# LLNL/MuyGPyS

Hardware: AMD Instinct MI355X
Metric: neighborhoods/sec (posterior mean+var) (higher is better)
Workload: dtype f32

## Files before the change

muygpys_amd/csrc/mgp_fused_wave_kernel.h:

```cpp
#pragma once

#include "mgp_wave_common.h"

#define MGP_PHASE(g, bit) ((g).mask & (bit))

#ifndef MGP_F64_SAME_PRIO
#define MGP_F64_SAME_PRIO 0
#endif
#ifndef MGP_DIST_PRIO
#define MGP_DIST_PRIO 1
#endif
#ifndef MGP_PRIO_EARLY_RAISE
#define MGP_PRIO_EARLY_RAISE 0
#endif
#ifndef MGP_W4
#define MGP_W4 0
#endif
#ifndef MGP_PRIO_LATE_DROP
#define MGP_PRIO_LATE_DROP 0
#endif
#ifndef MGP_XCHG_PRIO
#define MGP_XCHG_PRIO 0
#endif
#ifndef MGP_CHOL_PRIO
#define MGP_CHOL_PRIO 2
#endif
#ifndef MGP_LOOKAHEAD
#define MGP_LOOKAHEAD 1
#endif
#ifndef MGP_CHOL_ONE_BLOCK
#define MGP_CHOL_ONE_BLOCK 1
#endif
#ifndef MGP_F64_COV_BATCH
#define MGP_F64_COV_BATCH 5
#endif
#ifndef MGP_OWN_REG
#define MGP_OWN_REG 0
#endif
#ifndef MGP_C4_W3
#define MGP_C4_W3 1
#endif
#ifndef MGP_MODM
#define MGP_MODM 1
#endif
#ifndef MGP_GRAM
#define MGP_GRAM 1
#endif
#ifndef MGP_GRAM64
#define MGP_GRAM64 0
#endif
#ifndef MGP_DMA_ASM
#define MGP_DMA_ASM 1
#endif
#ifndef MGP_DIST_ASM
#define MGP_DIST_ASM 1
#endif
#ifndef MGP_F64_GC
#define MGP_F64_GC 6
#endif
#ifndef MGP_FOLD
#define MGP_FOLD 1
#endif
#ifndef MGP_DLT
#define MGP_DLT 1
#endif
#ifndef MGP_F64_DIST_HALF
#define MGP_F64_DIST_HALF 0
#endif

#ifndef MGP_BWD_COV_BATCH
#define MGP_BWD_COV_BATCH 3
#endif
#ifndef MGP_BWD_SWEEP_LATE
#define MGP_BWD_SWEEP_LATE -1
#endif
#ifndef MGP_BWD_EXP
#define MGP_BWD_EXP 0
#endif
#ifndef MGP_FEAT_EXP
#define MGP_FEAT_EXP 0
#endif

namespace mgp {

struct WaveGeom {
  int q;
  int dst;
  int xs;
  int vec_ok;
  int64_t ntasks;
  int mask;
  int gen_tab;
  float gen_h, gen_lc;
  double gen_h64, gen_lc64, gen_xmin64;
};

struct WaveDims {
  int E, CH, NH, NPL, NG, KS, KMAT, BA, BP, NS, M;
  bool STAT, TRI, MODM;
  bool DLT;
  int NR2, NPAIR, NSL;
};
constexpr int dlt_col_start(int c, int NR2) {
  const int m = c >> 1, b = c & 1;
  return 2 * m * NR2 - m * (m - 1) + b * (NR2 - m);
}
constexpr bool wave_bwd_tailfree(int es, int NP, bool gram, int dst) { return es == 4 && NP == 32 && gram && dst > 32 && dst <= 40; }
constexpr WaveDims wave_dims(int es, int NP, int KFIX, int RFIX, int DFIX, bool COEFF, bool GRAM) {
  WaveDims w{};
  w.E = 16 / es;
  w.CH = 2 * w.E;
  w.NH = 64 / NP;
  w.STAT = KFIX > 0 && RFIX > 0 && DFIX > 0 && !COEFF;
  w.NPL = w.STAT ? KFIX + 1 + RFIX : NP;
  w.NG = (w.NPL + w.E - 1) / w.E;
  w.KS = NP + w.E;
  w.TRI = NP == 64 && !COEFF;
  w.DLT = MGP_DLT && es == 8 && NP == 64 && w.STAT && RFIX >= 1;
  w.NR2 = (w.NPL + 1) / 2;
  w.NPAIR = dlt_col_start(w.NPL, w.NR2);
  w.NSL = (w.NPAIR + 63) / 64;
  w.KMAT = w.TRI ? w.E * ((w.NPL - 1) / w.E + 1) * (w.E * ((w.NPL - 1) / w.E) / 2 + (w.NPL - 1) % w.E) + w.NG * w.E + w.E
                 : NP * w.KS;
  if (w.DLT) w.KMAT = 2 * 64 * w.NSL + 2;
  w.M = NP;
  w.BA = 4;
  w.BP = NP / 8;
  w.MODM = false;
  if (MGP_MODM && w.STAT) {
    const int need = (KFIX + 1) / 2;
    int ba = 4, bp = (need + 3) / 4;
    for (int c = 3; c <= 5; c += 2) {
      const int q = (need + c - 1) / c;
      if (c * q < ba * bp) ba = c, bp = q;
    }
    if (ba * bp + (GRAM ? 2 : 1) <= NP / 2) {
      w.MODM = true;
      w.M = KFIX + 1;
      w.BA = ba;
      w.BP = bp;
    }
  }
  w.NS = w.BA * w.BP;
  return w;
}
constexpr int wave_pair_delta(int s, int BP, int M) {
  const int j = s / BP, p = s % BP + 1, o = j == 0 ? 0 : (j + 1) * BP + 1;
  return ((o - p) % M + M) % M;
}
constexpr bool wave_pair_first(int s, int BP, int M) {
  const int d = wave_pair_delta(s, BP, M);
  if (d == 0) return false;
  for (int t = 0; t < s; ++t) {
    const int e = wave_pair_delta(t, BP, M);
    if (e == d || e == M - d) return false;
  }
  return true;
}
constexpr unsigned long long wave_pair_first_mask(int NS, int BP, int M) {
  unsigned long long m = 0;
  for (int s = 0; s < NS; ++s)
    if (wave_pair_first(s, BP, M)) m |= 1ull << s;
  return m;
}
constexpr unsigned long long wave_pair_half_mask(int NS, int BP, int M) {
  unsigned long long m = 0;
  for (int s = 0; s < NS; ++s)
    if (2 * wave_pair_delta(s, BP, M) == M) m |= 1ull << s;
  return m;
}
constexpr int wave_tile_rows(const WaveDims& w, int NP, int KFIX, int xs) {
  if (!(w.STAT && w.NH == 1)) return w.NH * NP;
  const int spr = xs / w.E, pieces = ((KFIX + 1) * spr + 63) / 64;
  const int covered = (pieces * 64 + spr - 1) / spr;
  const int rows = w.MODM ? w.NPL : NP;
  return covered > rows ? covered : rows;
}
constexpr int wave_gather_pieces(const WaveDims& w, int KFIX, int xs) {
  const int spr = xs / w.E;
  return (w.STAT && w.NH == 1) ? ((KFIX + 1) * spr + 63) / 64 : spr;
}
constexpr int wave_stage_elems(const WaveDims& w) { return w.DLT ? 2 * (32 + 128) : 0; }
#ifndef MGP_RT_W3
#define MGP_RT_W3 1
#endif
constexpr int wave_min_waves(int es, int NP, int KFIX, int RFIX = 0, int DFIX = 0) {
  return es == 4 ? (NP <= 32 ? (KFIX == 30 && MGP_W4 ? 4 : 3) : (MGP_RT_W3 && KFIX == 0 ? 3 : 2))
                 : (NP <= 32 ? 2 : (MGP_C4_W3 && wave_dims(es, NP, KFIX, RFIX, DFIX, false, false).DLT ? 3 : 2));
}

#ifndef MGP_FOLD64
#define MGP_FOLD64 1
#endif
#ifndef MGP_FOLD16
#define MGP_FOLD16 0
#endif
#ifndef MGP_FOLD_F64
#define MGP_FOLD_F64 0
#endif
constexpr bool wave_fold(int es, int NP, int KFIX, int RFIX, int DFIX, bool PIPED, bool COEFF, bool GRAM) {
  return MGP_FOLD && PIPED && KFIX > 0 && RFIX >= 1 && DFIX > 0 && !COEFF && KFIX >= NP / 2 &&
         ((es == 4 && GRAM && (NP == 32 || (NP == 64 && MGP_FOLD64) || (NP == 16 && MGP_FOLD16))) || (es == 8 && NP == 32 && MGP_FOLD_F64));
}
constexpr int wave_colbuf_bytes(int es, int NP, bool fold) {
  const int need = fold ? (64 / (NP / 2)) * NP * es : 64 * es;
  return need > 512 ? need : 512;
}

template <int NPL_>
struct DltMeta {
  static constexpr int NR2 = (NPL_ + 1) / 2;
  static constexpr int NPAIR = dlt_col_start(NPL_, NR2);
  static constexpr int NSL = (NPAIR + 63) / 64;
  int rc[NSL * 64][2];
  constexpr DltMeta() : rc{} {
    int c = 0;
    for (int e = 0; e < NSL * 64; ++e) {
      while (c + 1 < NPL_ && dlt_col_start(c + 1, NR2) <= e) ++c;
      rc[e][0] = e < NPAIR ? 2 * (e - dlt_col_start(c, NR2) + (c >> 1)) : 0;
      rc[e][1] = c;
// ... 114 lines not shown
  const bool nopad = k == q;

  const int64_t ntasks = g.ntasks;
  const int64_t per_xcd = (ntasks + 7) / 8;
  const int xcd = blockIdx.x & 7;
  const int64_t t_hi = (xcd + 1) * per_xcd;
  const int64_t t_end = t_hi < ntasks ? t_hi : ntasks;
  const int64_t t_step = gridDim.x >> 3;

  auto load_index = [&](int task, int h, int i) -> int64_t {
    const int64_t nb0 = (int64_t)task * NH;
    const int hh = (NH > 1 && nb0 + h >= a.b) ? 0 : h;
    const int64_t* row = a.nn_idx + nb0 * k;
    const int64_t* p = row + (hh * k + (i < k ? i : 0));
    if (a.batch_idx != nullptr && i == q) p = a.batch_idx + nb0 + hh;
    return *p;
  };
  auto fix_index = [&](int64_t raw, int task, int h, int i) -> int64_t {
    const int64_t nb0 = (int64_t)task * NH;
    const int hh = (NH > 1 && nb0 + h >= a.b) ? 0 : h;
    if (i < k) return raw;
    if (i == q) return a.batch_idx != nullptr ? raw : nb0 + hh;
    return 0;
  };

  const int64_t task0 = xcd * per_xcd + (blockIdx.x >> 3);

  int g_pos = 0;
  auto seq_gen = [&]() -> int {
    const int64_t ts = task0 + (int64_t)g_pos * t_step;
    ++g_pos;
    return ts < t_end ? (int)ts : -1;
  };
  int task = seq_gen(), t1 = seq_gen(), t2 = -1;
  int64_t next_idx = 0;
  if (task >= 0) next_idx = load_index(task, NH == 1 ? 0 : (int)threadIdx.x / NP, threadIdx.x & (NP - 1));

  constexpr bool PIPE = PIPED;
  static_assert(!PIPED || DFIX <= DCAP, "the pipelined gather stages all features at once");
  const int SPR = xs / E;
  const int C16V = d / E;
  constexpr int GB = 11;
  const unsigned spr_magic = (1u << 20) / (unsigned)SPR + 1u;
  T pre_y = T(0), pre_eps = T(0);
  int64_t pre_idx = 0, pre_tg = 0;
  auto pipe_issue = [&](int task_n, int64_t idx_n, int lane_) {
    const int h = NH == 1 ? 0 : lane_ / NP;
    const int i = lane_ & (NP - 1);
    if constexpr (PACKED)
      rowaddr[lane_] = reinterpret_cast<const T*>(
          (i == q ? static_cast<const char*>(a.packed_q) + idx_n * a.q_stride
                  : static_cast<const char*>(a.packed_nn) + idx_n * a.nn_stride));
    else
      rowaddr[lane_] = (i == q ? feat_q : feat_nn) + idx_n * (int64_t)d;
    pre_idx = idx_n;
    __syncthreads();
    if (MGP_PHASE(g, 1)) {
      const int NPC = wave_gather_pieces(WD, KFIX, xs);
      for (int n0 = 0; n0 < NPC; n0 += GB) {
        const T* src[GB];
#pragma unroll
        for (int u = 0; u < GB; ++u) {
          if (n0 + u < NPC) {
            const unsigned sigma = 64u * (unsigned)(n0 + u) + (unsigned)lane_;
            const unsigned row = (sigma * spr_magic) >> 20;
            const unsigned c = min(sigma - row * (unsigned)SPR, (unsigned)(PACKED ? C16V : C16V - 1));
            src[u] = rowaddr[row] + c * E;
          }
        }
#pragma unroll
        for (int u = 0; u < GB; ++u)
          if (n0 + u < NPC) {
#if MGP_DMA_ASM
            glds16_asm(src[u], smem, (n0 + u) * 1024);
#else
            glds16_lds(src[u], smem, (n0 + u) * 1024);
#endif
          }
      }
    }
    {
      const int64_t nb0 = (int64_t)task_n * NH;
      const int hh = (NH > 1 && nb0 + h >= a.b) ? 0 : h;
      pre_tg = a.targets_batch ? (nb0 + hh) * k + (i < k ? i : 0) : (i < k ? idx_n : 0);
    }
    if (!PACKED || a.targets_batch) pre_y = targets[pre_tg * (int64_t)R];
    if constexpr (BWD) {
      if (a.R > 1) {
        const T* gmp = static_cast<const T*>(a.bwd_gmean);
        const int64_t nbq = (int64_t)task_n * NH + ((NH > 1 && (int64_t)task_n * NH + h >= a.b) ? 0 : h);
        T ys = T(0);
        for (int r = 0; r < a.R; ++r) ys = fma_t(gmp ? gmp[nbq * a.R + r] : T(0), targets[pre_tg * (int64_t)a.R + r], ys);
        pre_y = ys;
      }
    }
    pre_eps = (T)a.noise_scalar;
    if (a.noise_mode != MGP_NOISE_SCALAR) {
      const int64_t nb0 = (int64_t)task_n * NH;
      const int hh = (NH > 1 && nb0 + h >= a.b) ? 0 : h;
      const T* pn = a.noise_mode == MGP_NOISE_TABLE ? noise_dev + (i < k ? idx_n : 0) : noise_dev + nb0 * k + (hh * k + (i < k ? i : 0));
      pre_eps = *pn;
    }
  };
  if (PIPE && task >= 0) {
    pipe_issue(task, fix_index(next_idx, task, NH == 1 ? 0 : (int)threadIdx.x / NP, threadIdx.x & (NP - 1)),
               threadIdx.x);
    if (t1 >= 0) next_idx = load_index(t1, NH == 1 ? 0 : (int)threadIdx.x / NP, threadIdx.x & (NP - 1));
  }

  constexpr bool XPRE = (NP <= 32 || KFIX > 0) && !COEFF;
#ifndef MGP_FOLD_XPK
#define MGP_FOLD_XPK 0
#endif
#ifndef MGP_FOLD_DPRE
#define MGP_FOLD_DPRE 0
#endif
  constexpr bool XPK = XPRE && (NS > 16 || (FOLD && (MGP_FOLD_XPK || sizeof(T) == 8)));
  static_assert(!XPK || NH * KMAT + (BWD ? 4096 : 0) < 65536, "packed exchange offsets are 16-bit");
  int xoff[XPRE ? (XPK ? (NS + 1) / 2 : NS) : 1];
  unsigned xkeep = 0;
  if constexpr (XPRE) {
    const int i0 = threadIdx.x & (NP - 1);
    const int hbase = (NH == 1 ? 0 : (int)threadIdx.x / NP) * KMAT + kmat_base;
    const int dump0 = DLT ? KMAT - 2 : (TRI ? KMAT - E : (NP - 1) * KS + NP);
#pragma unroll
    for (int s = 1; s <= NS; ++s) {
      const int r1 = wrap(i0 + own_offset((s - 1) / BP));
      const int c = wrap(i0 + (s - 1) % BP + 1);
      const int hi = max(r1, c), lo = min(r1, c);
      const int xo = hbase + (hi <= q && hi != lo && i0 < M ? eoff(hi, lo) : dump0);
      if constexpr (XPK) {
        if ((s - 1) % 2 == 0) xoff[(s - 1) / 2] = xo;
        else xoff[(s - 1) / 2] |= xo << 16;
      } else {
        xoff[s - 1] = xo;
      }
      if (lo < k && (hi < k || hi == q)) xkeep |= 1u << (s - 1);
    }
  }

  constexpr bool DPRE = XPRE && DFIX > 0 && NP <= 32 && (!FOLD || MGP_FOLD_DPRE);
  int down[DPRE ? BA : 1], dpar[DPRE ? BP : 1];
  if constexpr (DPRE) {
    const int i0 = threadIdx.x & (NP - 1);
    const int hb = (NH == 1 ? 0 : (int)threadIdx.x / NP) * NP * xs;
#pragma unroll
    for (int j = 0; j < BA; ++j) down[j] = hb + wrap(i0 + own_offset(j)) * xs;
#pragma unroll
    for (int s2 = 1; s2 <= BP; ++s2) dpar[s2 - 1] = hb + wrap(i0 + s2) * xs;
  }
  static_assert(!MODM || XPRE, "the modulo-M pair scheme relies on the per-lane exchange offsets");
  static_assert(!DLT || XPRE, "the dealt layout is written through the per-lane exchange offsets");

  V FL[FOLD ? NG : 1], FS[FOLD ? NGS : 1];
  int fold_sub = 0;
  int fold_task_a = 0;
  for (; task >= 0; task = t1, t1 = t2) {
    int lane = threadIdx.x;
    asm volatile("" : "+v"(lane));
    const int h = NH == 1 ? 0 : lane / NP;
    const int i = lane & (NP - 1);
    T* Xh = tile + h * NP * xs;
    T* Kh = tile + kmat_base + h * KMAT;
    T* colh = TF ? Xh + KFIX * xs : colbuf + h * NP;
    int64_t* idxh = idxbuf + h * NP;
    const int64_t nb0 = (int64_t)task * NH;
    const bool live = nb0 + h < a.b;
    const int hh = live ? h : 0;


    int64_t myidx = 0, mytg = 0;
    T myeps = T(0), myy0 = T(0);
    V myyv = V(0);
    if (PIPE) {
      myidx = pre_idx;
      mytg = pre_tg;
      myy0 = i < k ? pre_y : T(0);
      myeps = pre_eps;
    } else {
      myidx = fix_index(next_idx, task, h, i);
      if (t1 >= 0) next_idx = load_index(t1, h, i);
      __syncthreads();
      idxh[i] = myidx * (int64_t)d;
      mytg = a.targets_batch ? (nb0 + hh) * k + (i < k ? i : 0) : myidx;
      if (i < k) {
        myy0 = targets[mytg * (int64_t)R];
        if (a.noise_mode == MGP_NOISE_SCALAR) myeps = (T)a.noise_scalar;
        else if (a.noise_mode == MGP_NOISE_TABLE) myeps = noise_dev[myidx];
        else myeps = (noise_dev + nb0 * k)[hh * k + i];
      }
    }

    ACC acc[NS];
#pragma unroll
    for (int s = 0; s < NS; ++s) acc[s] = ACC(0);
#if MGP_CHOL_PRIO && MGP_PRIO_LATE_DROP
    __builtin_amdgcn_s_setprio(0);
#endif
#if MGP_DIST_PRIO
    __builtin_amdgcn_s_setprio(sizeof(T) == 4 || MGP_F64_SAME_PRIO ? MGP_DIST_PRIO : MGP_XCHG_PRIO);
#endif

    for (int d0 = 0; d0 < d; d0 += dst) {
      const int w = min(dst, d - d0);
      const int wp = (w + CH - 1) / CH * CH;
      constexpr int ILN = PIPED ? (DSTFIX + 63) / 64 : 1;
      T il_pre[ILN];
      if constexpr (PIPED) {
#pragma unroll
        for (int u = 0; u < ILN; ++u) {
          const int c = u * 64 + lane;
          il_pre[u] = (aniso && c < w) ? T(1) / ls[d0 + c] : T(0);
        }
      }
#if MGP_DMA_ASM
      if (PIPE) lds_dma_wait();
#endif
      __syncthreads();
      MGP_WAVE_T(0)
      if (PIPE) {
        if constexpr (PACKED) {
          if (!a.targets_batch) {
            myyv = *reinterpret_cast<const V*>(Xh + (NPL == NP ? i : min(i, NPL - 1)) * xs + d);
            myy0 = i < k ? myyv[0] : T(0);
          }
        }
        if (wp > w && (NPL == NP || i < NPL)) *reinterpret_cast<V*>(Xh + i * xs + w) = V(0);
      } else if (!MGP_PHASE(g, 1)) {
      } else if (DFIX > 0 || g.vec_ok) {
        const int c16 = w / E, c16p = wp / E;
        const int rpr = NP / c16p;
        const int sub = DFIX > 0 ? i / c16p : (int)(((unsigned)i * ((1u << 16) / (unsigned)c16p + 1u)) >> 16);
        const int c = i - sub * c16p;
        const bool lane_on = sub < rpr;
        constexpr int RPRFIX = NP / (DSTFIX / E);
        constexpr int U = (KFIX > 0 && DFIX > 0) ? (KFIX + RPRFIX - 1) / RPRFIX : 6;
        const int64_t* idxl = idxh + sub;
        T* xdst = Xh + sub * xs + c * E;
        for (int r0 = 0; r0 < k; r0 += U * rpr) {
          V v[U];
#pragma unroll
          for (int u = 0; u < U; ++u) {
            const int row = r0 + u * rpr + sub;
            v[u] = V(0);
            if (lane_on && row < k && c < c16)
              v[u] = *reinterpret_cast<const V*>(feat_nn + idxl[r0 + u * rpr] + d0 + c * E);
          }
#pragma unroll
          for (int u = 0; u < U; ++u) {
            const int row = r0 + u * rpr + sub;
            if (lane_on && row < k) *reinterpret_cast<V*>(xdst + (r0 + u * rpr) * xs) = v[u];
          }
        }
        if (i < c16p) {
          V vq = V(0);
          if (i < c16) vq = *reinterpret_cast<const V*>(feat_q + idxh[q] + d0 + i * E);
          *reinterpret_cast<V*>(Xh + q * xs + i * E) = vq;
        }
        if (!nopad)
          for (int t = i; t < (q - k) * c16p; t += NP) {
            const int row = k + t / c16p;
            *reinterpret_cast<V*>(Xh + row * xs + (t % c16p) * E) = V(0);
          }
      } else {
        const unsigned magic = (1u << 20) / (unsigned)wp + 1u;
        for (int t = i; t < NP * wp; t += NP) {
          const int row = (int)(((unsigned)t * magic) >> 20);
          const int c = t - row * wp;
          T v = T(0);
          if (c < w && (row < k || row == q)) v = ((row < k ? feat_nn : feat_q) + idxh[row] + d0)[c];
          Xh[row * xs + c] = v;
        }
      }
      if (aniso) {
        if constexpr (PIPED) {
#pragma unroll
          for (int u = 0; u < ILN; ++u)
            if (u * 64 + lane < wp) ilbuf[u * 64 + lane] = il_pre[u];
        } else {
          for (int c = lane; c < wp; c += 64) ilbuf[c] = c < w ? T(1) / ls[d0 + c] : T(0);
        }
      }
      __syncthreads();

      if constexpr (GRAM) {
        constexpr bool NDUP = sizeof(T) == 4;
        constexpr int NCYC = MODM ? M : NP;
        T* nrmh = (TF ? tile + kmat_base : colbuf) + h * (NDUP ? 2 * NP : NP);
        const int iw = MODM ? wrap(i) : i;
        auto put_norm = [&](bool has, T n2) {
          if (MODM && !has) return;
          const T v = has ? n2 : num<T>::inf();
          nrmh[iw] = v;
          if constexpr (NDUP) nrmh[iw + NCYC] = v;
        };
        constexpr int NCF = DFIX > 0 ? DSTFIX / E : 1;
        constexpr bool OWNREG = MGP_OWN_REG && DFIX > 0;
        V x[DFIX > 0 ? NCF : 1];
        if (MGP_PHASE(g, 2)) {
          const bool has = i < k || i == q;
          T* xrow = Xh + (MODM ? wrap(i) : i) * xs;
          const T* qrow = Xh + q * xs;
          if constexpr (DFIX > 0 && (FOLD || (BWD && NCF > 16)) && NCF > 10 && !OWNREG) {
            ACC n4[4] = {ACC(0), ACC(0), ACC(0), ACC(0)};
#pragma unroll
            for (int c0 = 0; c0 < NCF; c0 += 4) {
              V xc[4], qc[4];
#pragma unroll
              for (int u = 0; u < 4; ++u)
                if (c0 + u < NCF) {
                  xc[u] = *reinterpret_cast<const V*>(xrow + (c0 + u) * E);
                  qc[u] = *reinterpret_cast<const V*>(qrow + (c0 + u) * E);
                }
#pragma unroll
              for (int u = 0; u < 4; ++u)
                if (c0 + u < NCF) {
                  xc[u] = vsub(xc[u], qc[u]);
                  if (aniso) xc[u] = xc[u] * *reinterpret_cast<const V*>(ilbuf + (c0 + u) * E);
                  norm_accum(n4[u], xc[u]);
                }
              if (has) {
#pragma unroll
                for (int u = 0; u < 4; ++u)
                  if (c0 + u < NCF) *reinterpret_cast<V*>(xrow + (c0 + u) * E) = xc[u];
              }
              __builtin_amdgcn_sched_barrier(0);
            }
            const ACC n2 = (n4[0] + n4[1]) + (n4[2] + n4[3]);
            put_norm(has, acc_total(n2));
          } else if constexpr (DFIX > 0) {
            V qv[NCF];
#pragma unroll
            for (int c = 0; c < NCF; ++c) {
              x[c] = *reinterpret_cast<const V*>(xrow + c * E);
              qv[c] = *reinterpret_cast<const V*>(qrow + c * E);
            }
#pragma unroll
            for (int c = 0; c < NCF; ++c) {
              x[c] = vsub(x[c], qv[c]);
              if (aniso) x[c] = x[c] * *reinterpret_cast<const V*>(ilbuf + c * E);
            }
            if (has) {
#pragma unroll
              for (int c = 0; c < NCF; ++c) *reinterpret_cast<V*>(xrow + c * E) = x[c];
            }
            ACC n4[4] = {ACC(0), ACC(0), ACC(0), ACC(0)};
#pragma unroll
            for (int c = 0; c < NCF; ++c) norm_accum(n4[c & 3], x[c]);
            const ACC n2 = (n4[0] + n4[1]) + (n4[2] + n4[3]);
            put_norm(has, acc_total(n2));
          } else {
            ACC n2 = ACC(0);
            for (int c0 = 0; c0 < wp; c0 += CH) {
              V x0 = *reinterpret_cast<const V*>(xrow + c0), x1 = *reinterpret_cast<const V*>(xrow + c0 + E);
              const V q0 = *reinterpret_cast<const V*>(qrow + c0), q1 = *reinterpret_cast<const V*>(qrow + c0 + E);
              x0 = vsub(x0, q0);
              x1 = vsub(x1, q1);
              if (aniso) {
                x0 = x0 * *reinterpret_cast<const V*>(ilbuf + c0);
                x1 = x1 * *reinterpret_cast<const V*>(ilbuf + c0 + E);
              }
              norm_accum(n2, x0);
              norm_accum(n2, x1);
              if (has) {
                *reinterpret_cast<V*>(xrow + c0) = x0;
                *reinterpret_cast<V*>(xrow + c0 + E) = x1;
              }
            }
            put_norm(has, acc_total(n2));
          }
        }
        __syncthreads();
        MGP_WAVE_T(1)
        if (MGP_PHASE(g, 2)) {
#pragma unroll
          for (int c0 = 0; c0 < (DFIX > 0 ? DSTFIX : wp); c0 += CH) {
            V own0[BA], own1[BA];
#pragma unroll
            for (int j = 0; j < BA; ++j) {
              if (OWNREG && j == 0) {
                own0[0] = x[OWNREG ? c0 / E : 0];
                own1[0] = x[OWNREG ? c0 / E + 1 : 0];
                continue;
              }
              const T* xj = DPRE ? tile + down[DPRE ? j : 0] + c0 : Xh + wrap(i + own_offset(j)) * xs + c0;
              own0[j] = *reinterpret_cast<const V*>(xj);
              own1[j] = *reinterpret_cast<const V*>(xj + E);
            }
#pragma unroll
            for (int s = 1; s <= BP; ++s) {
              const T* xo = DPRE ? tile + dpar[DPRE ? s - 1 : 0] + c0 : Xh + wrap(i + s) * xs + c0;
              const V o0 = *reinterpret_cast<const V*>(xo);
              const V o1 = *reinterpret_cast<const V*>(xo + E);
              gram_block<BA, BP>(&acc[s - 1], own0, o0);
              gram_block<BA, BP>(&acc[s - 1], own1, o1);
            }
          }
          T nown[BA];
#pragma unroll
          for (int j = 0; j < BA; ++j) nown[j] = NDUP ? nrmh[iw + own_offset(j)] : nrmh[wrap(i + own_offset(j))];
          T guard = T(1);
#pragma unroll
          for (int s = 0; s < BP; ++s) {
            const T np1 = NDUP ? nrmh[iw + s + 1] : nrmh[wrap(i + s + 1)];
#pragma unroll
            for (int j = 0; j + 1 < BA; j += 2)
              gram_finish2(acc[j * BP + s], acc[(j + 1) * BP + s], nown[j] + np1, nown[j + 1] + np1, guard);
            if constexpr (BA % 2 == 1) gram_finish1(acc[(BA - 1) * BP + s], nown[BA - 1] + np1, guard);
          }
          const unsigned long long tripped = gram_guard_lanes(guard);
          if (tripped != 0) {
            const bool mine = NH == 1 || ((tripped >> (h * NP)) & ((NP == 32 ? 0xFFFFFFFFull : 0xFFFFull))) != 0;
            const int ngrp = (DFIX > 0 ? DSTFIX : wp) / E;
            if (mine) {
#pragma unroll
              for (int s = 0; s < NS; ++s) {
                const T* xa = DPRE ? tile + down[DPRE ? s / BP : 0] : Xh + wrap(i + own_offset(s / BP)) * xs;
                const T* xb = DPRE ? tile + dpar[DPRE ? s % BP : 0] : Xh + wrap(i + s % BP + 1) * xs;
                ACC sum = ACC(0);
#pragma nounroll
                for (int c = 0; c < ngrp; ++c)
                  accum(sum, vsub(*reinterpret_cast<const V*>(xa + c * E), *reinterpret_cast<const V*>(xb + c * E)));
                gram_from_diff(sum);
                acc[s] = sum;
              }
            }
          }
        }
      } else
      if (MGP_PHASE(g, 2)) {
        if (aniso) {
          if (i < k || i == q) {
            T* xrow = Xh + i * xs;
            for (int c0 = 0; c0 < wp; c0 += E) {
              V x = *reinterpret_cast<const V*>(xrow + c0);
              x = x * *reinterpret_cast<const V*>(ilbuf + c0);
              *reinterpret_cast<V*>(xrow + c0) = x;
            }
          }
          __syncthreads();
        }
        if constexpr (sizeof(T) == 8 && MGP_F64_DIST_HALF) {
#pragma unroll
          for (int c0 = 0; c0 < (DFIX > 0 ? DSTFIX : wp); c0 += E) {
            V own[BA];
#pragma unroll
            for (int j = 0; j < BA; ++j)
              own[j] = *reinterpret_cast<const V*>((DPRE ? tile + down[DPRE ? j : 0] : Xh + wrap(i + own_offset(j)) * xs) + c0);
#pragma unroll
            for (int s = 1; s <= BP; ++s) {
              const V o = *reinterpret_cast<const V*>((DPRE ? tile + dpar[DPRE ? s - 1 : 0] : Xh + wrap(i + s) * xs) + c0);
#pragma unroll
              for (int j = 0; j < BA; ++j) accum(acc[j * BP + s - 1], vsub(own[j], o));
            }
            if (MGP_F64_DIST_HALF == 2) __builtin_amdgcn_sched_barrier(0);
          }
        } else {
#pragma unroll
          for (int c0 = 0; c0 < (DFIX > 0 ? DSTFIX : wp); c0 += CH) {
            V own0[BA], own1[BA];
#pragma unroll
            for (int j = 0; j < BA; ++j) {
              const T* xj = DPRE ? tile + down[DPRE ? j : 0] + c0 : Xh + wrap(i + own_offset(j)) * xs + c0;
              own0[j] = *reinterpret_cast<const V*>(xj);
              own1[j] = *reinterpret_cast<const V*>(xj + E);
            }
#pragma unroll
            for (int s = 1; s <= BP; ++s) {
              const T* xo = DPRE ? tile + dpar[DPRE ? s - 1 : 0] + c0 : Xh + wrap(i + s) * xs + c0;
              const V o0 = *reinterpret_cast<const V*>(xo);
              const V o1 = *reinterpret_cast<const V*>(xo + E);
              if constexpr (sizeof(T) == 4 && BA == 4 && MGP_DIST_ASM) {
                dist_block4(acc[s - 1], acc[BP + s - 1], acc[2 * BP + s - 1], acc[3 * BP + s - 1], own0[0], own0[1],
                            own0[2], own0[3], o0);
                dist_block4(acc[s - 1], acc[BP + s - 1], acc[2 * BP + s - 1], acc[3 * BP + s - 1], own1[0], own1[1],
                            own1[2], own1[3], o1);
              } else {
#pragma unroll
                for (int j = 0; j < BA; ++j) {
                  accum(acc[j * BP + s - 1], vsub(own0[j], o0));
                  accum(acc[j * BP + s - 1], vsub(own1[j], o1));
                }
              }
            }
          }
        }
      }
    }

    MGP_WAVE_T(2)
#if MGP_XCHG_PRIO || MGP_DIST_PRIO
    __builtin_amdgcn_s_setprio(sizeof(T) == 4 || MGP_F64_SAME_PRIO ? MGP_XCHG_PRIO : MGP_DIST_PRIO);
#endif
    __syncthreads();
    V A[DLT ? 1 : NG];
    V Dp[DLT ? NSL : 1];
    int wrow[DLT ? NSL : 1], wcol[DLT ? NSL : 1];
    {
      int i3 = i;
      asm volatile("" : "+v"(i3));
      T* Kh3 = tile + kmat_base + (NH == 1 ? 0 : (lane / NP) * KMAT);
      if (MGP_PHASE(g, 4)) {
        const int dump = TRI ? KMAT - E : (NP - 1) * KS + NP;
        auto put = [&](int s, T v) {
          if constexpr (XPRE) {
            if (!nopad) v = (xkeep >> (s - 1)) & 1u ? v : T(0);
            if constexpr (XPK) tile[(s - 1) % 2 == 0 ? (xoff[(s - 1) / 2] & 0xFFFF) : ((unsigned)xoff[(s - 1) / 2] >> 16)] = v;
            else tile[xoff[s - 1]] = v;
          } else {
            const int r1 = wrap(i3 + own_offset((s - 1) / BP));
            const int c = wrap(i3 + (s - 1) % BP + 1);
            const int hi = max(r1, c), lo = min(r1, c);
            if (!nopad) v = (lo < k && (hi < k || hi == q)) ? v : T(0);
            Kh3[hi <= q && hi != lo ? rowoff(hi) + lo : dump] = v;
          }
        };
        auto covariances = [&](auto kid, auto mid) {
          constexpr int KID = decltype(kid)::value, MID = decltype(mid)::value;
          if constexpr (KID == MGP_KERNEL_MATERN_GEN) {
            if constexpr (sizeof(T) == 4 && XPRE) {
              float kv[NS];
#pragma unroll
              for (int s = 0; s < NS; ++s) {
                float sqd;
                if constexpr (GRAM) sqd = gram_sq(acc[s]);
                else sqd = acc_total(acc[s]);
                kv[s] = (MID == MGP_METRIC_L2 ? sqrt_fast(sqd) : sqd) * post_scale;
              }
              matern_gen_eval<NS>(kv, xkeep, gtab, (float)a.smoothness, g.gen_h, g.gen_lc);
#pragma unroll
              for (int s = 1; s <= NS; ++s) put(s, kv[s - 1]);
            } else if constexpr (sizeof(T) == 8 && XPRE) {
#ifndef MGP_F64_GEN_BATCH
#define MGP_F64_GEN_BATCH 3
#endif
              constexpr int CB = MGP_F64_GEN_BATCH;
              const double* gtab64 = reinterpret_cast<const double*>(smem + g.gen_tab);
              unsigned keep = 0;
#pragma unroll
              for (int s = 1; s <= NS; ++s) {
                const int r1 = wrap(i3 + own_offset((s - 1) / BP)), c = wrap(i3 + (s - 1) % BP + 1);
                const int hi = max(r1, c), lo = min(r1, c);
                if (lo < k && (hi < k || hi == q) && hi != lo) keep |= 1u << (s - 1);
              }
#pragma unroll
              for (int s0 = 0; s0 < NS; s0 += CB) {
                double kv[CB];
#pragma unroll
                for (int u = 0; u < CB; ++u) {
                  const int su = s0 + u < NS ? s0 + u : NS - 1;
                  kv[u] = GRAM ? gram_sq(acc[su]) : acc_total(acc[su]);
                }
                metric_batch64<CB, MID>(kv, post_scale);
                matern_gen_batch64<CB>(kv, (keep >> s0) & ((1u << CB) - 1u), gtab64, a.smoothness, g.gen_h64, g.gen_lc64,
                                       g.gen_xmin64);
#pragma unroll
                for (int u = 0; u < CB; ++u)
                  if (s0 + u < NS) put(s0 + u + 1, kv[u]);
                __builtin_amdgcn_sched_barrier(0);
              }
            }
          } else if constexpr (sizeof(T) == 4) {
            T kv[NS];
            auto sq = [&](int s) {
              if constexpr (GRAM) return gram_sq(acc[s]);
              else return acc_total(acc[s]);
            };
#pragma unroll
            for (int s = 0; s + 1 < NS; s += 2) {
              const f2 kk = cov_from_sqdist2(f2{sq(s), sq(s + 1)}, KID, MID, post_scale);
              kv[s] = kk.x;
              kv[s + 1] = kk.y;
            }
            if constexpr (NS % 2 == 1) kv[NS - 1] = cov_from_sqdist<T>(sq(NS - 1), KID, MID, post_scale);
#pragma unroll
            for (int s = 1; s <= NS; ++s) put(s, kv[s - 1]);
          } else {
            constexpr int CB = BWD ? MGP_BWD_COV_BATCH : MGP_F64_COV_BATCH;
#pragma unroll
            for (int s0 = 0; s0 < NS; s0 += CB) {
              T kv[CB];
#ifndef MGP_COV_BATCH64
#define MGP_COV_BATCH64 1
#endif
              if constexpr (sizeof(T) == 8 && MGP_COV_BATCH64) {
#pragma unroll
                for (int u = 0; u < CB; ++u) {
                  const int su = s0 + u < NS ? s0 + u : NS - 1;
                  kv[u] = GRAM ? gram_sq(acc[su]) : acc_total(acc[su]);
                }
                cov_batch64<CB, KID, MID>(kv, post_scale);
              } else {
#pragma unroll
              for (int u = 0; u < CB; ++u)
                if (s0 + u < NS) kv[u] = cov_from_sqdist<T>(GRAM ? gram_sq(acc[s0 + u]) : acc_total(acc[s0 + u]), KID, MID, post_scale);
              }
#pragma unroll
              for (int u = 0; u < CB; ++u)
                if (s0 + u < NS) put(s0 + u + 1, kv[u]);
              __builtin_amdgcn_sched_barrier(0);
            }
          }
        };
        if constexpr (GEN64) {
          if (a.metric_id == MGP_METRIC_L2) covariances(ic<MGP_KERNEL_MATERN_GEN>{}, ic<MGP_METRIC_L2>{});
          else covariances(ic<MGP_KERNEL_MATERN_GEN>{}, ic<MGP_METRIC_F2>{});
        } else if constexpr (sizeof(T) == 4) {
          kernel_dispatch_gen(a.kernel_id, a.metric_id, covariances);
        } else {
          kernel_dispatch(a.kernel_id, a.metric_id, covariances);
        }
      }
      if (NPL == NP || i3 < NPL) Kh3[eoff(i3, i3)] = i3 < k ? T(1) + myeps : (i3 <= q ? T(1) : T(0));
      if (!TRI || i3 <= q + 1) Kh3[eoff(q + 1, i3)] = myy0;
      if (PACKED && !a.targets_batch) {
#pragma unroll
        for (int r = 1; r < E; ++r)
          if (r < R && (!TRI || i3 <= q + 1 + r)) Kh3[eoff(q + 1 + r, i3)] = i3 < k ? myyv[r] : T(0);
      } else {
        for (int r = 1; r < R; ++r)
          if (!TRI || i3 <= q + 1 + r) Kh3[eoff(q + 1 + r, i3)] = i3 < k ? targets[mytg * (int64_t)R + r] : T(0);
      }
    }
    __syncthreads();
#if MGP_CHOL_PRIO && MGP_PRIO_EARLY_RAISE
    __builtin_amdgcn_s_setprio(MGP_CHOL_PRIO);
#endif
    if constexpr (FOLD) {
      if ((lane >> 5) == fold_sub) {
        const T* Kq = tile + (NH == 1 ? 0 : (lane >> LOGH) & (NH - 1)) * KMAT;
        const int lh = lane & (HALF - 1);
#pragma unroll
        for (int c4 = 0; c4 < NGS; ++c4) FS[c4] = *reinterpret_cast<const V*>(Kq + rowoff(lh) + c4 * E);
#pragma unroll
        for (int c4 = 0; c4 < NG; ++c4) FL[c4] = *reinterpret_cast<const V*>(Kq + rowoff(HALF + lh) + c4 * E);
      }
    } else if constexpr (DLT) {
#pragma unroll
      for (int s = 0; s < NSL; ++s) {
        typedef int i2 __attribute__((ext_vector_type(2)));
        const i2 m = *reinterpret_cast<const i2*>(&g_dlt_meta<DLT ? NPL : 2>.rc[64 * s + lane][0]);
        wrow[s] = m.x;
        wcol[s] = m.y;
      }
#pragma unroll
      for (int s = 0; s < NSL; ++s) Dp[s] = *reinterpret_cast<const V*>(Kh + 2 * (64 * s) + 2 * lane);
    } else {
      const T* myrow = Kh + rowoff(NPL == NP ? i : min(i, NPL - 1));
#pragma unroll
      for (int c4 = 0; c4 < NG; ++c4) A[c4] = *reinterpret_cast<const V*>(myrow + c4 * E);
    }

    t2 = seq_gen();
    if (PIPE && !BWD && t1 >= 0) {
      pipe_issue(t1, fix_index(next_idx, t1, h, i), lane);
      if (t2 >= 0) next_idx = load_index(t2, h, i);
    }

    if constexpr (FOLD) {
      const bool lastt = t1 < 0;
      MGP_WAVE_T(3)
      if (fold_sub == 0 && !lastt) {
        fold_sub = 1;
        fold_task_a = task;
        continue;
      }
      const bool have_b = fold_sub == 1;
      if (!have_b) fold_task_a = task;
      fold_sub = 0;
      bool bad = false;
#if MGP_CHOL_PRIO
      __builtin_amdgcn_s_setprio(MGP_CHOL_PRIO);
#endif
      if (MGP_PHASE(g, 8)) {
        const int lh = lane & (HALF - 1);
        T* colq = colbuf + (lane >> LOGH) * NP;
        if constexpr (sizeof(T) == 4) {
          colq[HALF + lh] = FL[0][0];
          colq[lh] = FS[0][0];
          V piv = *reinterpret_cast<const V*>(colq);
#pragma unroll
          for (int j = 0; j < KFIX; ++j) {
            const int g0 = j / E, e0 = j % E;
            const bool sh = j < HALF;
            const T aL = FL[g0][e0];
            const T aS = sh ? FS[g0 < NGS ? g0 : 0][e0] : T(0);
            V col[NG];
            col[g0] = piv;
#pragma unroll
            for (int c4 = g0 + 1; c4 < NG; ++c4) col[c4] = *reinterpret_cast<const V*>(colq + c4 * E);
            const T p = piv[e0];
            bad = bad || !(p > T(0));
            const T rp = pivot_rcp(p);
            const V ntL = V(-aL * rp), ntS = V(-aS * rp);
            const int g1 = (j + 1 < KFIX ? j + 1 : j) / E;
            FL[g1] = col[g1] * ntL + FL[g1];
            if (sh && g1 < NGS) FS[g1] = col[g1] * ntS + FS[g1];
            if (j + 1 < KFIX) {
              colq[HALF + lh] = FL[g1][(j + 1) % E];
              if (j + 1 < HALF) colq[lh] = FS[g1][(j + 1) % E];
              piv = *reinterpret_cast<const V*>(colq + g1 * E);
            }
#pragma unroll
            for (int c4 = g0; c4 < NG; ++c4)
              if (c4 != g1) FL[c4] = col[c4] * ntL + FL[c4];
            if (sh) {
#pragma unroll
              for (int c4 = g0; c4 < NGS; ++c4)
                if (c4 != g1) FS[c4] = col[c4] * ntS + FS[c4];
            }
          }
        } else {
#pragma unroll
          for (int j = 0; j < KFIX; ++j) {
            const int g0 = j / E, e0 = j % E;
            const bool sh = j < HALF;
            const T aL = FL[g0][e0];
            const T aS = sh ? FS[g0 < NGS ? g0 : 0][e0] : T(0);
            colq[HALF + lh] = aL;
            if (sh) colq[lh] = aS;
            const V cp = *reinterpret_cast<const V*>(colq + g0 * E);
            const T p = cp[e0];
            bad = bad || !(p > T(0));
            const T rp = pivot_rcp(p);
            const V ntL = V(-aL * rp), ntS = V(-aS * rp);
            FL[g0] = cp * ntL + FL[g0];
            if (sh) FS[g0 < NGS ? g0 : 0] = cp * ntS + FS[g0 < NGS ? g0 : 0];
            constexpr int GC = MGP_F64_GC;
#pragma unroll
            for (int c0 = g0 + 1; c0 < NG; c0 += GC) {
              V cv[GC];
#pragma unroll
              for (int u = 0; u < GC; ++u)
                if (c0 + u < NG) cv[u] = *reinterpret_cast<const V*>(colq + (c0 + u) * E);
#pragma unroll
              for (int u = 0; u < GC; ++u)
                if (c0 + u < NG) {
                  FL[c0 + u] = cv[u] * ntL + FL[c0 + u];
                  if (sh && c0 + u < NGS) FS[c0 + u] = cv[u] * ntS + FS[c0 + u];
                }
            }
          }
        }
      }
#if MGP_CHOL_PRIO
      __builtin_amdgcn_s_setprio(0);
#endif
      MGP_WAVE_T(4)
      if constexpr (RFIX > 1) {
        constexpr int QF = KFIX;
        const int l16 = lane & (HALF - 1);
        const bool second = (lane >> 5) != 0;
        const int64_t nbq = (int64_t)(second ? task : fold_task_a) * NH + (NH == 1 ? 0 : (lane >> LOGH) & (NH - 1));
        const bool liveq = nbq < a.b && (!second || have_b);
        T* mean = static_cast<T*>(a.mean);
        T* var = static_cast<T*>(a.var);
        T* yk = static_cast<T*>(a.ykinvy);
        const T sq = FL[QF / E][QF % E];
        T sd = T(0);
        if (yk) {
#pragma unroll
          for (int c = QF + 1; c < NG * E; ++c) sd = c == HALF + l16 ? FL[c / E][c % E] : sd;
        }
        if (liveq) {
          if (l16 == QF - HALF) {
            *(var + nbq) = bad ? num<T>::nan() : sq;
            if (bad && a.info) atomicAdd(a.info, 1);
          } else if (l16 > QF - HALF && l16 <= QF - HALF + RFIX) {
            const int r = l16 - (QF - HALF) - 1;
            *(mean + (nbq * RFIX + r)) = bad ? num<T>::nan() : -sq;
            if (yk) *(yk + (nbq * RFIX + r)) = bad ? num<T>::nan() : -sd;
          }
        }
      } else {
        constexpr int QF = KFIX, YF = KFIX + 1;
        const int l16 = lane & (HALF - 1);
        const bool second = (lane >> 5) != 0;
        const int64_t nbq = (int64_t)(second ? task : fold_task_a) * NH + (NH == 1 ? 0 : (lane >> LOGH) & (NH - 1));
        const bool liveq = nbq < a.b && (!second || have_b);
        T* mean = static_cast<T*>(a.mean);
        T* var = static_cast<T*>(a.var);
        T* yk = static_cast<T*>(a.ykinvy);
        const T sq = FL[QF / E][QF % E], sy = FL[YF / E][YF % E];
        if (liveq) {
          if (l16 == QF - HALF) {
            *(var + nbq) = bad ? num<T>::nan() : sq;
            if (bad && a.info) atomicAdd(a.info, 1);
          } else if (l16 == YF - HALF) {
            *(mean + nbq) = bad ? num<T>::nan() : -sq;
            if (yk) *(yk + nbq) = bad ? num<T>::nan() : -sy;
          }
        }
      }
      MGP_WAVE_T(5)
      continue;
    }
    if constexpr (DLT) {
      MGP_WAVE_T(3)
      bool bad = false;
#if MGP_CHOL_PRIO
      __builtin_amdgcn_s_setprio(MGP_CHOL_PRIO);
#endif
      if (MGP_PHASE(g, 8)) {
        T* stg = tile + tile_rows * xs + 64;
        T nrp = T(0);
        unsigned badm = 0;
        auto post = [&](int j) {
          const int ep = cs2(j);
          const int s0 = ep >> 6, s1 = (cs2(j + 1) - 1) >> 6;
#pragma unroll
          for (int s = s0; s <= s1; ++s) *reinterpret_cast<V*>(stg + 2 * (64 * (s - s0)) + 2 * lane) = Dp[s];
          if constexpr (BWD && !(MGP_BWD_EXP & 8)) {
#pragma unroll
            for (int s = s0; s <= s1; ++s) {
              T* dstp = wcol[s] == j ? Kh + 2 * (64 * s) + 2 * lane : stg + 2 * (64 * (s - s0)) + 2 * lane;
              *reinterpret_cast<V*>(dstp) = Dp[s];
            }
          }
          const long long pb = __double_as_longlong(Dp[s0][j & 1]);
          const unsigned plo = __builtin_amdgcn_readlane((int)(pb & 0xFFFFFFFFll), ep & 63);
          const unsigned phi = __builtin_amdgcn_readlane((int)(pb >> 32), ep & 63);
          badm = max(badm, phi - 1u);
          nrp = -pivot_rcp(__longlong_as_double(((long long)phi << 32) | plo));
        };
        post(0);
#pragma unroll
        for (int j = 0; j < KFIX; ++j) {
          const T nrpj = nrp;
          const int cj = 2 * (cs2(j) - 64 * (cs2(j) >> 6) - (j >> 1));
          const int sl = cs2(j + 1) >> 6;
#ifndef MGP_DLT_CHUNK
#define MGP_DLT_CHUNK 0
#endif
          constexpr int CHK = MGP_DLT_CHUNK > 0 ? MGP_DLT_CHUNK : (DFIX <= 8 && KFIX <= 52 ? 2 : 4);
          const int n1 = j + 1 < KFIX ? (cs2(j + 2) - 1) >> 6 : sl - 1;
#pragma unroll
          for (int sc = sl; sc < NSL; sc += CHK) {
            V wp[CHK];
            T wc[CHK];
#pragma unroll
            for (int u = 0; u < CHK; ++u)
              if (sc + u < NSL) {
                wp[u] = *reinterpret_cast<const V*>(stg + cj + wrow[sc + u]);
                wc[u] = (stg + cj)[wcol[sc + u]];
              }
            auto update = [&](int u) {
              const T ngq = wc[u] * nrpj;
              Dp[sc + u][0] = fma_t(wp[u][0], ngq, Dp[sc + u][0]);
              Dp[sc + u][1] = fma_t(wp[u][1], ngq, Dp[sc + u][1]);
            };
            const bool last_chunk = sc + CHK >= NSL;
#pragma unroll
            for (int u = 0; u < CHK; ++u)
              if (sc + u < NSL && sc + u <= n1) update(u);
            if (last_chunk && j + 1 < KFIX) post(j + 1);
#pragma unroll
            for (int u = 0; u < CHK; ++u)
              if (sc + u < NSL && sc + u > n1) update(u);
          }
        }
        bad = badm >= 0x7FEFFFFFu;
      }
#if MGP_CHOL_PRIO
      __builtin_amdgcn_s_setprio(0);
#endif
      MGP_WAVE_T(4)
      if constexpr (BWD) {
        __syncthreads();
        const T* Lh = Kh;
        const int ic = i < KFIX ? i : KFIX - 1;
        const int lbase = 2 * (cs2(ic) - (ic >> 1));
        const T rp = pivot_rcp(Lh[lbase + ic]);
        T xa = i < KFIX ? Lh[lbase + KFIX] * rp : T(0);
        T xu = i < KFIX ? Lh[lbase + KFIX + 1] * rp : T(0);
        if (!(MGP_BWD_EXP & 4)) {
          constexpr int BB = 8;
#pragma unroll
          for (int mb = (KFIX - 1) / BB * BB; mb >= 0; mb -= BB) {
            T lm[BB];
#pragma unroll
            for (int e = 0; e < BB; ++e)
              if (mb + e >= 1 && mb + e < KFIX) lm[e] = Lh[lbase + mb + e];
#pragma unroll
            for (int e = BB - 1; e >= 0; --e) {
              const int m = mb + e;
              if (m >= 1 && m < KFIX) {
                const T am = lane_value(xa, m), um = lane_value(xu, m);
                const T t = i < m ? lm[e] * rp : T(0);
                xa = fma_t(-t, am, xa);
                xu = fma_t(-t, um, xu);
              }
            }
          }
        }
        T* avec = tile + tile_rows * xs;
        T* uvec = avec + 64;
        __syncthreads();
        avec[lane] = i < KFIX ? xa : (i == KFIX ? T(-1) : T(0));
        uvec[lane] = i < KFIX ? xu : T(0);
        __syncthreads();
        const T gmv = (live && a.bwd_gmean) ? (a.R > 1 ? T(1) : static_cast<const T*>(a.bwd_gmean)[nb0]) : T(0);
        const T gvv = (live && a.bwd_gvar) ? static_cast<const T*>(a.bwd_gvar)[nb0] : T(0);
// ... 596 lines not shown
```

Baseline: 637.8 million.

## Add mirrored fold register layout and software-prefetched Gram loop

For f32 fold kernels with NP=32, the separate long-row and short-row register arrays are replaced by a single mirrored array (FM). Each lane holds long-row groups and short-row tail groups in shared registers, which lowers register pressure and skips needless column loads during the in-register Cholesky, with a matching output path. The Gram distance loop also gets an explicit software-pipelined path that prefetches partner-row vectors a few steps ahead and double-buffers own-row loads, with sched_barriers to fix the ordering. This is intended to hide LDS latency, at the cost of complex index logic that could be wrong in edge cases and of more live registers from the prefetch buffers.

```diff
diff --git a/muygpys_amd/csrc/mgp_fused_wave_kernel.h b/muygpys_amd/csrc/mgp_fused_wave_kernel.h
--- a/muygpys_amd/csrc/mgp_fused_wave_kernel.h
+++ b/muygpys_amd/csrc/mgp_fused_wave_kernel.h
@@ -66,6 +66,9 @@
 #endif
 #ifndef MGP_F64_DIST_HALF
 #define MGP_F64_DIST_HALF 0
+#endif
+#ifndef MGP_GRAM_PREFETCH
+#define MGP_GRAM_PREFETCH 3
 #endif
 
 #ifndef MGP_BWD_COV_BATCH
@@ -486,7 +489,10 @@
   static_assert(!MODM || XPRE, "the modulo-M pair scheme relies on the per-lane exchange offsets");
   static_assert(!DLT || XPRE, "the dealt layout is written through the per-lane exchange offsets");
 
-  V FL[FOLD ? NG : 1], FS[FOLD ? NGS : 1];
+  constexpr bool MIRROR = FOLD && sizeof(T) == 4 && NP == 32;
+  constexpr int NGM = (NP + 1 + E - 1) / E;
+  static_assert(!MIRROR || (NG >= 5 && NG <= 8), "mirror fold: registers 0 .. 4 hold long-row groups in every lane");
+  V FL[FOLD && !MIRROR ? NG : 1], FS[FOLD && !MIRROR ? NGS : 1], FM[MIRROR ? NGM : 1];
   int fold_sub = 0;
   int fold_task_a = 0;
   for (; task >= 0; task = t1, t1 = t2) {
@@ -630,6 +636,7 @@
         };
         constexpr int NCF = DFIX > 0 ? DSTFIX / E : 1;
         constexpr bool OWNREG = MGP_OWN_REG && DFIX > 0;
+        constexpr bool GPF = FOLD && sizeof(T) == 4 && DFIX > 0 && !OWNREG && !DPRE && MGP_GRAM_PREFETCH > 0;
         V x[DFIX > 0 ? NCF : 1];
         if (MGP_PHASE(g, 2)) {
           const bool has = i < k || i == q;
@@ -707,6 +714,29 @@
         __syncthreads();
         MGP_WAVE_T(1)
         if (MGP_PHASE(g, 2)) {
+          if constexpr (GPF) {
+            constexpr int NGR = DSTFIX / E, NT = NGR * BP, GPD = MGP_GRAM_PREFETCH;
+            auto own_row = [&](int j) { return Xh + wrap(i + own_offset(j)) * xs; };
+            auto par_group = [&](int t) { return *reinterpret_cast<const V*>(Xh + wrap(i + t % BP + 1) * xs + (t / BP) * E); };
+            V own[2][BA], par[GPD + 1];
+#pragma unroll
+            for (int j = 0; j < BA; ++j) own[0][j] = *reinterpret_cast<const V*>(own_row(j));
+#pragma unroll
+            for (int t = 0; t < GPD && t < NT; ++t) par[t] = par_group(t);
+            __builtin_amdgcn_sched_barrier(0);
+#pragma unroll
+            for (int t = 0; t < NT; ++t) {
+              const int gi = t / BP, s = t % BP;
+              if (t + GPD < NT) par[(t + GPD) % (GPD + 1)] = par_group(t + GPD);
+              if (s == 0 && gi + 1 < NGR) {
+#pragma unroll
+                for (int j = 0; j < BA; ++j) own[(gi + 1) & 1][j] = *reinterpret_cast<const V*>(own_row(j) + (gi + 1) * E);
+              }
+              __builtin_amdgcn_sched_barrier(0);
+              gram_block<BA, BP>(&acc[s], own[gi & 1], par[t % (GPD + 1)]);
+              __builtin_amdgcn_sched_barrier(0);
+            }
+          } else {
 #pragma unroll
           for (int c0 = 0; c0 < (DFIX > 0 ? DSTFIX : wp); c0 += CH) {
             V own0[BA], own1[BA];
@@ -729,6 +759,7 @@
               gram_block<BA, BP>(&acc[s - 1], own0, o0);
               gram_block<BA, BP>(&acc[s - 1], own1, o1);
             }
+          }
           }
           T nown[BA];
 #pragma unroll
@@ -964,10 +995,21 @@
       if ((lane >> 5) == fold_sub) {
         const T* Kq = tile + (NH == 1 ? 0 : (lane >> LOGH) & (NH - 1)) * KMAT;
         const int lh = lane & (HALF - 1);
-#pragma unroll
-        for (int c4 = 0; c4 < NGS; ++c4) FS[c4] = *reinterpret_cast<const V*>(Kq + rowoff(lh) + c4 * E);
-#pragma unroll
-        for (int c4 = 0; c4 < NG; ++c4) FL[c4] = *reinterpret_cast<const V*>(Kq + rowoff(HALF + lh) + c4 * E);
+        if constexpr (MIRROR) {
+          const T* rS = Kq + rowoff(lh);
+          const T* rL = Kq + rowoff(NP - 1 - lh);
+#pragma unroll
+          for (int r = 0; r < NGM; ++r) {
+            const int sg = NGM - 1 - r;
+            const T* src = r <= 4 ? rL + r * E : (r == NGM - 1 || r >= NG ? rS + sg * E : (lh >= E * sg ? rS + sg * E : rL + r * E));
+            FM[r] = *reinterpret_cast<const V*>(src);
+          }
+        } else {
+#pragma unroll
+          for (int c4 = 0; c4 < NGS; ++c4) FS[c4] = *reinterpret_cast<const V*>(Kq + rowoff(lh) + c4 * E);
+#pragma unroll
+          for (int c4 = 0; c4 < NG; ++c4) FL[c4] = *reinterpret_cast<const V*>(Kq + rowoff(HALF + lh) + c4 * E);
+        }
       }
     } else if constexpr (DLT) {
 #pragma unroll
@@ -1009,7 +1051,65 @@
       if (MGP_PHASE(g, 8)) {
         const int lh = lane & (HALF - 1);
         T* colq = colbuf + (lane >> LOGH) * NP;
-        if constexpr (sizeof(T) == 4) {
+        if constexpr (MIRROR) {
+          constexpr int NMX = 3;
+          bool shm[NMX];
+          const T* cmx[NMX];
+#pragma unroll
+          for (int u = 0; u < NMX; ++u) {
+            const int r = 5 + u, sg = NGM - 1 - r;
+            shm[u] = lh >= E * sg;
+            cmx[u] = colq + (shm[u] ? sg : r) * E;
+          }
+          auto kind = [](int r, int j) {
+            const int g0 = j / E, sg = NGM - 1 - r;
+            const bool la = r < NG && r >= g0 && r < NGM - 1, sa = r > 4 && j < HALF && sg >= g0;
+            return la && sa ? 3 : (la ? 1 : (sa ? 2 : 0));
+          };
+          colq[NP - 1 - lh] = FM[0][0];
+          colq[lh] = FM[NGM - 1][0];
+          V piv = *reinterpret_cast<const V*>(colq);
+#pragma unroll
+          for (int j = 0; j < KFIX; ++j) {
+            const int g0 = j / E, e0 = j % E;
+            const bool sh = j < HALF;
+            const T aL = FM[g0][e0];
+            const T aS = sh ? FM[NGM - 1 - g0][e0] : T(0);
+            V col[NG], colm[NMX];
+            col[g0] = piv;
+#pragma unroll
+            for (int c4 = g0 + 1; c4 < NG; ++c4) {
+              const bool need = kind(c4, j) == 1 || (NGM - 1 - c4 > 4 && kind(NGM - 1 - c4, j) == 2);
+              if (need) col[c4] = *reinterpret_cast<const V*>(colq + c4 * E);
+            }
+#pragma unroll
+            for (int u = 0; u < NMX; ++u)
+              if (kind(5 + u, j) == 3) colm[u] = *reinterpret_cast<const V*>(cmx[u]);
+            const T p = piv[e0];
+            bad = bad || !(p > T(0));
+            const T rp = pivot_rcp(p);
+            const T nL = -aL * rp, nS = -aS * rp;
+            const V ntL = V(nL), ntS = V(nS);
+            auto upd = [&](int r) {
+              const int kd = kind(r, j);
+              if (kd == 1) FM[r] = col[r < NG ? r : 0] * ntL + FM[r];
+              else if (kd == 2) FM[r] = col[NGM - 1 - r] * ntS + FM[r];
+              else if (kd == 3) FM[r] = colm[r - 5] * V(shm[r - 5] ? nS : nL) + FM[r];
+            };
+            const int g1 = (j + 1 < KFIX ? j + 1 : j) / E;
+            const int s1 = j + 1 < HALF ? NGM - 1 - g1 : -1;
+            upd(g1);
+            if (s1 >= 0) upd(s1);
+            if (j + 1 < KFIX) {
+              colq[NP - 1 - lh] = FM[g1][(j + 1) % E];
+              if (s1 >= 0) colq[lh] = FM[s1][(j + 1) % E];
+              piv = *reinterpret_cast<const V*>(colq + g1 * E);
+            }
+#pragma unroll
+            for (int r = 0; r < NGM; ++r)
+              if (r != g1 && r != s1) upd(r);
+          }
+        } else if constexpr (sizeof(T) == 4) {
           colq[HALF + lh] = FL[0][0];
           colq[lh] = FS[0][0];
           V piv = *reinterpret_cast<const V*>(colq);
@@ -1081,7 +1181,33 @@
       __builtin_amdgcn_s_setprio(0);
 #endif
       MGP_WAVE_T(4)
-      if constexpr (RFIX > 1) {
+      if constexpr (MIRROR) {
+        constexpr int QF = KFIX;
+        const int l16 = lane & (HALF - 1);
+        const int row = NP - 1 - l16;
+        const bool second = (lane >> 5) != 0;
+        const int64_t nbq = (int64_t)(second ? task : fold_task_a) * NH + (NH == 1 ? 0 : (lane >> LOGH) & (NH - 1));
+        const bool liveq = nbq < a.b && (!second || have_b);
+        T* mean = static_cast<T*>(a.mean);
+        T* var = static_cast<T*>(a.var);
+        T* yk = static_cast<T*>(a.ykinvy);
+        const T sq = FM[QF / E][QF % E];
+        T sd = T(0);
+        if (yk) {
+#pragma unroll
+          for (int c = QF + 1; c < QF + 1 + RFIX; ++c) sd = c == row ? FM[c / E][c % E] : sd;
+        }
+        if (liveq) {
+          if (row == QF) {
+            *(var + nbq) = bad ? num<T>::nan() : sq;
+            if (bad && a.info) atomicAdd(a.info, 1);
+          } else if (row > QF && row <= QF + RFIX) {
+            const int r = row - QF - 1;
+            *(mean + (nbq * RFIX + r)) = bad ? num<T>::nan() : -sq;
+            if (yk) *(yk + (nbq * RFIX + r)) = bad ? num<T>::nan() : -sd;
+          }
+        }
+      } else if constexpr (RFIX > 1) {
         constexpr int QF = KFIX;
         const int l16 = lane & (HALF - 1);
         const bool second = (lane >> 5) != 0;
```

After: 652.9 million, median of 6. +2.4%, better.
